# hG3n/mvStereoVision3

Measured on AMD Instinct MI355X. Metric: Mpix disparities/sec (SGBM 128-disp, 8-path) at 1/2/4/8 GPUs; % HBM roofline, higher is better.
Workload: dtype int16; 1 GPU; sgbm_1280x960_d128_8path_batch8; width=1280, height=960, num_disparities=128, min_disparity=1, block_size=13, mode=MODE_HH, frames_per_gpu=8, global_batch=8, params=configs/sgbm.yml + mode, gather=none, launch=single process, batches_in_flight=2, parallelism=frame-parallel x1

## Files before the change

mvstereovision3_amd/csrc/mvsv_bsgm.hip:

```cpp
#include <algorithm>
#include <cstdio>
#include <cstdlib>
#include <cstring>
#include <type_traits>
#include <vector>

#include "mvsv_bitslice.hpp"
#include "mvsv_device.hpp"
#include "mvsv_internal.hpp"

namespace mvsv {

using namespace dev;

namespace {

constexpr uint32_t kOnes = 0xffffffffu;

__device__ __forceinline__ uint32_t xswap(uint32_t v)
{
    return (uint32_t)__builtin_amdgcn_mov_dpp((int)v, 0xB1, 0xf, 0xf, true);
}

template <int P1, int P2>
// ... 571 lines not shown
        const int xl = x - dlo, xh = x - dhi;
        auto d2at = [&](int xx) -> int {
            const uint32_t kk = __hip_atomic_load(krow + xx, __ATOMIC_RELAXED, __HIP_MEMORY_SCOPE_AGENT);
            if (kk == 0xffffffffu) return INV;
            const int xc = 0xffff - (int)(kk & 0xffffu);
            return xc + minX1 - xx;
        };
        if (0 <= xl && xl < W && 0 <= xh && xh < W) {
            const int a = d2at(xl), b = d2at(xh);
            if (a >= minD && abs(a - dlo) > e.disp12 && b >= minD && abs(b - dhi) > e.disp12)
                orow[x] = (int16_t)INV;
        }
    }
}

constexpr int kBsWtaThreads = 512;

template <bool SIDE, int NDIR>
__global__ __launch_bounds__(kBsWtaThreads) void bsgm_wta_kernel(const uint32_t* __restrict__ Bc,
                                                                 const uint32_t* __restrict__ A, size_t aplane,
                                                                 const uint32_t* __restrict__ Dl, size_t dplane,
                                                                 const int16_t* __restrict__ C,
                                                                 const uint16_t* __restrict__ Mv, int H, int W,
                                                                 SgbmEff e, int16_t* __restrict__ raw,
                                                                 uint32_t* __restrict__ keys)
{
    static_assert(NDIR == 8 || NDIR == 5, "8 or 5 directions");
    const int y = blockIdx.x, f = blockIdx.y;
    const int W1 = e.W1;
    const int INV = e.invalid;
    const bool lane_rule = NDIR == 5 && !(e.variant & MVSV_VARIANT_WTA_MIN_D);
    int16_t* orow = raw + ((size_t)f * H + y) * W;
    uint32_t* krow = keys + ((size_t)f * H + y) * W;
    for (int x = threadIdx.x; x < W; x += kBsWtaThreads) {
        orow[x] = (int16_t)INV;
        krow[x] = 0xffffffffu;
    }
    __threadfence_block();
    __syncthreads();
    const int h = threadIdx.x & 1;
    const size_t pix0 = ((size_t)f * H + y) * W1;
    for (int xb = 0; xb < W1; xb += kBsWtaThreads / 2) {
        const int xr = xb + (threadIdx.x >> 1);
        const bool own = xr < W1;
        const int x = min(xr, W1 - 1);
        const size_t pix = pix0 + x;
        uint32_t c[2][4];
        uint32_t S[2][7];
        const size_t rowq = (size_t)(f * H + y) * bs::padq(W1);
        const uint32_t* qc = Bc + bs::cq_word(rowq, x, 2 * h);
        if constexpr (SIDE) {
#pragma unroll
            for (int e2 = 0; e2 < 2; e2++) {
                const uint4 t = *(const uint4*)(qc + 16 * e2);
                c[e2][0] = t.x, c[e2][1] = t.y, c[e2][2] = t.z, c[e2][3] = t.w;
                uint32_t dd[NDIR][3];
#pragma unroll
                for (int i = 0; i < NDIR; i++) {
                    const uint32_t* qd = Dl + (size_t)i * dplane + bs::dl_word(rowq, x, 2 * h + e2);
#pragma unroll
                    for (int b = 0; b < 3; b++) dd[i][b] = qd[b];
                }
                uint32_t a4[4][4], a5[2][5], s6[6];
                bs::add33(dd[0], dd[1], a4[0]);
                bs::add33(dd[2], dd[3], a4[1]);
                bs::add44(a4[0], a4[1], a5[0]);
                if constexpr (NDIR == 8) {
                    bs::add33(dd[4], dd[5], a4[2]);
                    bs::add33(dd[6], dd[7], a4[3]);
                    bs::add44(a4[2], a4[3], a5[1]);
                    bs::add55(a5[0], a5[1], s6);
                    bs::total8(c[e2], s6, S[e2]);
                } else {
                    const uint32_t d4[4] = {dd[4][0], dd[4][1], dd[4][2], 0u};
                    bs::add54(a5[0], d4, s6);
                    const uint32_t s5[5] = {s6[0], s6[1], s6[2], s6[3], s6[4]};
                    bs::total5(c[e2], s5, S[e2]);
                }
            }
        } else {
            const uint4* qd = (const uint4*)(A + pix * 16 + h * 8);
            const uint4* qu = (const uint4*)(A + aplane + pix * 16 + h * 8);
            const uint32_t* ql = Dl + bs::dl_word(rowq, x, 2 * h);
            const uint32_t* qr = Dl + dplane + bs::dl_word(rowq, x, 2 * h);
#pragma unroll
            for (int e2 = 0; e2 < 2; e2++) {
                uint4 t = *(const uint4*)(qc + 16 * e2);
                c[e2][0] = t.x, c[e2][1] = t.y, c[e2][2] = t.z, c[e2][3] = t.w;
                uint32_t ad[4], dl[3], dr[3];
                t = qd[e2];
                ad[0] = t.x, ad[1] = t.y, ad[2] = t.z, ad[3] = t.w;
#pragma unroll
                for (int b = 0; b < 3; b++) {
                    dl[b] = ql[12 * e2 + b];
                    dr[b] = qr[12 * e2 + b];
                }
                uint32_t d4[4];
                bs::add33(dl, dr, d4);
                if constexpr (NDIR == 8) {
                    uint32_t au[4], s5[5], s6[6];
                    t = qu[e2];
                    au[0] = t.x, au[1] = t.y, au[2] = t.z, au[3] = t.w;
                    bs::add44(ad, au, s5);
                    bs::add54(s5, d4, s6);
                    bs::total8(c[e2], s6, S[e2]);
                } else {
                    uint32_t s5[5];
                    bs::add44(ad, d4, s5);
                    bs::total5(c[e2], s5, S[e2]);
                }
            }
        }
        constexpr int TOP = NDIR == 8 ? 5 : 4;
        uint32_t kE = NDIR == 8 ? ~S[0][6] : ~(S[0][6] | S[0][5]);
        uint32_t kO = NDIR == 8 ? ~S[1][6] : ~(S[1][6] | S[1][5]);
        int mins = 0;
#pragma unroll
        for (int b = TOP; b >= 0; b--) {
            const uint32_t zE = bs::lop3<bs::kAndNotAB>(S[0][b], kE, kE);
            const uint32_t zO = bs::lop3<bs::kAndNotAB>(S[1][b], kO, kO);
            uint32_t any = zE | zO;
            any |= xswap(any);
            const bool fz = any != 0u;
            kE = fz ? zE : kE;
            kO = fz ? zO : kO;
            mins |= fz ? 0 : 1 << b;
        }
        int key = min(bs::wta_key(kE, h, 0, lane_rule), bs::wta_key(kO, h, 1, lane_rule));
        key = min(key, (int)xswap((uint32_t)key));
        const int best = key & 127;
        const int eb = best & 1;
        int Sm = 0, Sp = 0;
        {
            const int pm = ((best - 1 - 64 * h) >> 1) & 31, pp = ((best + 1 - 64 * h) >> 1) & 31;
#pragma unroll
            for (int b = 0; b < 7; b++) {
                const uint32_t wv = eb ? S[0][b] : S[1][b];
                Sm |= (int)(__builtin_amdgcn_ubfe(wv, (uint32_t)pm, 1u) << b);
                Sp |= (int)(__builtin_amdgcn_ubfe(wv, (uint32_t)pp, 1u) << b);
            }
            const int Smo = (int)xswap((uint32_t)Sm), Spo = (int)xswap((uint32_t)Sp);
            if (((best - 1) >> 6) != h) Sm = Smo;
            if (((best + 1) >> 6) != h) Sp = Spo;
        }
        if (h == 0 && own) bs_finish_pixel(C, Mv, pix, W1, W, x, best, mins, Sm, Sp, e, orow, krow);
    }
    __threadfence_block();
    __syncthreads();
    bs_lr_check_row(orow, krow, W, e, kBsWtaThreads);
}

constexpr int kBsRG = 3;

template <int P1, int P2, int NDIR>
__global__ __launch_bounds__(64) void bsgm_rlwta_kernel(const uint32_t* __restrict__ Bc,
                                                         const uint32_t* __restrict__ A, size_t aplane,
                                                         const uint32_t* __restrict__ Dlr, int H, int W1,
                                                         uint32_t* __restrict__ rec, int lane_rule)
{
    static_assert(NDIR == 8 || NDIR == 5, "8 or 5 directions");
    const int lane = threadIdx.x;
    const int q = lane & 3, rr = lane >> 2;
    const int y = min((int)blockIdx.x * 16 + rr, H - 1);
    const int f = blockIdx.y;
    const int h = q >> 1, eo = q & 1;
    const bool odd = eo != 0;
    const uint32_t fill_hi = q == 3 ? kOnes : 0u, fill_lo = q == 0 ? kOnes : 0u, sh = odd ? 1u : 31u;
    const size_t rowq = (size_t)(f * H + y) * bs::padq(W1);
    const size_t pixrow = (size_t)(f * H + y) * W1;
    const uint4* cgrp = (const uint4*)(Bc + bs::cq_word(rowq, 0, q));
    const uint4* dgrp = (const uint4*)(Dlr + bs::dl_word(rowq, 0, q));
    const uint4* adn = (const uint4*)(A + pixrow * 16 + 4 * q);
    const uint4* aup = (const uint4*)(A + aplane + pixrow * 16 + 4 * q);
    uint4* rgrp = (uint4*)(rec + rowq);
    const int G = (W1 + 3) >> 2;
    const int part = W1 & 3;
    auto grp = [&](int i) { return max(G - 1 - i, 0); };
    struct Ops {
        uint4 c[4], d[3], a[4], b[4];
    };
    auto load = [&](Ops& o, int i) {
        const int g = grp(i);
#pragma unroll
        for (int u = 0; u < 4; u++) o.c[u] = cgrp[(size_t)g * 16 + u];
#pragma unroll
        for (int u = 0; u < 3; u++) o.d[u] = dgrp[(size_t)g * 12 + u];
#pragma unroll
        for (int u = 0; u < 4; u++) {
            const int x = min(4 * g + u, W1 - 1);
            o.a[u] = adn[(size_t)x * 4];
            if constexpr (NDIR == 8) o.b[u] = aup[(size_t)x * 4];
        }
    };
    const int ph = part ? 1 : 0;
    Ops c0, ring[kBsRG];
    if (ph) load(c0, 0);
#pragma unroll
    for (int j = 0; j < kBsRG; j++) {
        load(ring[j], ph + j);
        __builtin_amdgcn_sched_barrier(0);
    }
    uint32_t st[3] = {0u, 0u, 0u};
    auto w4 = [](const uint4& v, int i) { return i == 0 ? v.x : i == 1 ? v.y : i == 2 ? v.z : v.w; };
    auto group = [&](int i, Ops& o, int n) {
        uint32_t rv[4];
#pragma unroll
        for (int k = 0; k < 4; k++) {
            const int u = 3 - k;
            if (u < n) {
                const uint32_t cw[4] = {o.c[u].x, o.c[u].y, o.c[u].z, o.c[u].w};
                uint32_t nw[3], dr[3];
                bs_quad_step<P1, P2>(st, cw, fill_hi, fill_lo, odd, sh, nw, dr);
#pragma unroll
                for (int b = 0; b < 3; b++) st[b] = nw[b];
                const uint32_t ad[4] = {o.a[u].x, o.a[u].y, o.a[u].z, o.a[u].w};
                uint32_t dl[3];
#pragma unroll
                for (int b = 0; b < 3; b++) dl[b] = w4(o.d[(3 * u + b) >> 2], (3 * u + b) & 3);
                uint32_t d4[4], S[7];
                bs::add33(dl, dr, d4);
                if constexpr (NDIR == 8) {
                    const uint32_t au[4] = {o.b[u].x, o.b[u].y, o.b[u].z, o.b[u].w};
                    uint32_t s5[5], s6[6];
                    bs::add44(ad, au, s5);
                    bs::add54(s5, d4, s6);
                    bs::total8(cw, s6, S);
                } else {
                    uint32_t s5[5];
                    bs::add44(ad, d4, s5);
                    bs::total5(cw, s5, S);
                }
                constexpr int TOP = NDIR == 8 ? 5 : 4;
                uint32_t kk = NDIR == 8 ? ~S[6] : ~(S[6] | S[5]);
                int mins = 0;
#pragma unroll
                for (int b = TOP; b >= 0; b--) {
                    const uint32_t z = bs::lop3<bs::kAndNotAB>(S[b], kk, kk);
                    uint32_t any = z | xswap(z);
                    any |= (uint32_t)__builtin_amdgcn_mov_dpp((int)any, 0x4E, 0xf, 0xf, true);
                    const bool fz = any != 0u;
                    kk = fz ? z : kk;
                    mins |= fz ? 0 : 1 << b;
                }
                int key = bs::wta_key(kk, h, eo, NDIR == 5 && lane_rule);
                key = min(key, (int)xswap((uint32_t)key));
                key = min(key, __builtin_amdgcn_mov_dpp(key, 0x4E, 0xf, 0xf, true));
                const int best = key & 127;
                auto sat = [&](int d) -> uint32_t {
                    const int dq = 2 * ((d >> 6) & 1) + (d & 1), p = ((d & 63) >> 1);
                    uint32_t v = 0;
#pragma unroll
                    for (int b = 0; b < 7; b++) v |= __builtin_amdgcn_ubfe(S[b], (uint32_t)p, 1u) << b;
                    return dq == q ? v : 0u;
                };
                uint32_t sm = sat(best - 1) | (sat(best + 1) << 8);
                sm |= xswap(sm);
                sm |= (uint32_t)__builtin_amdgcn_mov_dpp((int)sm, 0x4E, 0xf, 0xf, true);
                rv[u] = (uint32_t)best | ((uint32_t)mins << 8) | (sm << 16);
            } else {
                rv[u] = 0u;
            }
        }
        rgrp[grp(i)] = make_uint4(rv[0], rv[1], rv[2], rv[3]);
    };
    auto ringstep = [&](int i, int j, int n) {
        group(i, ring[j], n);
        load(ring[j], i + kBsRG);
        __builtin_amdgcn_sched_barrier(0);
    };
    if (ph) group(0, c0, part);
    int i = ph;
    for (; i + kBsRG <= G; i += kBsRG) {
#pragma unroll
        for (int j = 0; j < kBsRG; j++) ringstep(i + j, j, 4);
    }
#pragma unroll
    for (int j = 0; j < kBsRG; j++)
        if (i + j < G) ringstep(i + j, j, 4);
}

constexpr int kBsFinThreads = 256;
__global__ __launch_bounds__(kBsFinThreads) void bsgm_rl_final_kernel(const uint32_t* __restrict__ rec,
                                                                      const int16_t* __restrict__ C,
                                                                      const uint16_t* __restrict__ Mv, int H, int W,
                                                                      SgbmEff e, int16_t* __restrict__ raw,
                                                                      uint32_t* __restrict__ keys)
{
    const int y = blockIdx.x, f = blockIdx.y;
    const int W1 = e.W1;
    int16_t* orow = raw + ((size_t)f * H + y) * W;
    uint32_t* krow = keys + ((size_t)f * H + y) * W;
    for (int x = threadIdx.x; x < W; x += kBsFinThreads) {
        orow[x] = (int16_t)e.invalid;
        krow[x] = 0xffffffffu;
    }
    __threadfence_block();
    __syncthreads();
    const uint32_t* rrow = rec + (size_t)(f * H + y) * bs::padq(W1);
    const size_t pix0 = ((size_t)f * H + y) * W1;
    for (int x = threadIdx.x; x < W1; x += kBsFinThreads) {
        const uint32_t r = rrow[x];
        bs_finish_pixel(C, Mv, pix0 + x, W1, W, x, (int)(r & 0xffu), (int)((r >> 8) & 0xffu),
                        (int)((r >> 16) & 0xffu), (int)(r >> 24), e, orow, krow);
    }
    __threadfence_block();
    __syncthreads();
    bs_lr_check_row(orow, krow, W, e, kBsFinThreads);
}

__global__ __launch_bounds__(256) void bsgm_fixup_bottom_kernel(uint32_t* __restrict__ Bc, int16_t* __restrict__ C,
                                                                uint16_t* __restrict__ Mv, int H, int W1, int ylast,
                                                                int ybot)
{
    const int y = ybot + blockIdx.y, f = blockIdx.z;
    const size_t W1q = (size_t)bs::padq(W1);
    const size_t i = (size_t)blockIdx.x * 256 + threadIdx.x;
    const size_t nb = W1q * 4, nc = W1q * 16;
    const size_t src = (size_t)f * H + ylast, dst = (size_t)f * H + y;
    if (i < nb) {
        ((uint4*)Bc)[dst * nb + i] = ((const uint4*)Bc)[src * nb + i];
    } else if (i < nb + nc) {
        const size_t j = i - nb;
        ((uint4*)C)[dst * nc + j] = ((const uint4*)C)[src * nc + j];
    }
    if (i < (size_t)W1) Mv[dst * W1 + i] = Mv[src * W1 + i];
}

__global__ __launch_bounds__(128) void bsgm_fixup_col0_kernel(uint32_t* __restrict__ Bc, int16_t* __restrict__ C,
                                                              uint16_t* __restrict__ Mv, int H, int W1)
{
    const int y = 1 + blockIdx.x, f = blockIdx.y;
    const size_t W1q = (size_t)bs::padq(W1);
    const size_t r0 = (size_t)f * H, r = r0 + y;
    const int t = threadIdx.x;
    if (t < 16) {
        const int o = (t >> 2) * 16 + (t & 3);
        Bc[bs::cq_word(r * W1q, 0, 0) + o] = Bc[bs::cq_word(r0 * W1q, 0, 0) + o];
    }
    C[(r * W1q) * 128 + t * 4] = C[(r0 * W1q) * 128 + t * 4];
    if (t == 0) Mv[r * W1] = Mv[r0 * W1];
}

}

template <int NG>
static int launch_bs_strips(mvsv_ctx* ctx, const SgbmPlan& plan, int n, int H, const SgbmEff& e, const uint32_t* Bv,
                            uint32_t* Av, size_t aplane, uint32_t* dummy)
{
    using Cfg = BsStripCfg<NG>;
    int rc;
    unsigned epoch;
    long long ticket0;
    if ((rc = strip_begin(ctx, ctx->bs_bnd, 32, &epoch, &ticket0))) return rc;
    const dim3 grid((unsigned)plan.blocks);
    unsigned long long* stats = ctx->opt.bs_stats ? strip_stats_alloc(ctx, (size_t)grid.x * 64) : nullptr;
    const size_t lds = std::max(Cfg::kBytes, (size_t)(ctx->opt.bs_ldspad >= 0 ? ctx->opt.bs_ldspad : kBsStripLds));
    if (lds > 65536 &&
        (rc = check_hip(ctx, hipFuncSetAttribute((const void*)bsgm_strip_kernel<NG, 2, 5>,
                                                 hipFuncAttributeMaxDynamicSharedMemorySize, (int)lds),
                        "bit-sliced strip LDS attribute")))
        return rc;
    hipLaunchKernelGGL((bsgm_strip_kernel<NG, 2, 5>), grid, dim3(Cfg::kThreads), lds, ctx->stream, Bv, Av,
                       aplane, dummy, H, e.W1, plan.passes, (unsigned long long*)ctx->bs_bnd.ptr, epoch, n,
                       (int*)ctx->status.ptr, ctx->opt.spin_limit, ctx->report_target, ticket0, stats, 0);
    rc = check_hip(ctx, hipGetLastError(), "bit-sliced strip kernel");
    if (rc == MVSV_OK && ticket0 >= 0) ctx->tri_tickets += grid.x;
    std::vector<unsigned long long> hv;
    if (stats && strip_stats_read(ctx, stats, (size_t)grid.x * 8, &hv)) {
        unsigned long long t0 = ~0ull, t1 = 0, spin = 0, busy = 0, steps = 0;
        for (size_t b = 0; b < grid.x; b++) {
            const unsigned long long* q = &hv[b * 8];
            if (!q[1]) continue;
            t0 = std::min(t0, q[0]);
            t1 = std::max(t1, q[1]);
            spin += q[2];
            busy += q[1] - q[0];
            steps += q[4];
        }
        std::fprintf(stderr, "[bs] NG %d strips %d blocks %u span %llu ticks, block-ticks %llu, spin %.1f%%, ticks/step %.1f\n",
                     NG, plan.nstrips, grid.x, t1 - t0, busy, 100.0 * spin / std::max(busy, 1ull),
                     (double)busy / std::max(steps, 1ull));
    }
    return rc;
}

static int bsgm_paths_side(mvsv_ctx* ctx, const SgbmPlan& plan, int n, int H, int W, const SgbmEff& e,
                           const int16_t* Cv, const uint32_t* Bv, const uint16_t* Mv, int16_t* raw)
{
    int rc;
    const int npass = e.fullDP ? 2 : 1, ndir = plan.nplanes;
    const size_t dplane = plan.bs_dplane;
    uint32_t* Dv = (uint32_t*)ctx->agg.ptr;
    hipStream_t s = ctx->stream;
    {
        StageTimer tm(ctx, kStagePath);
        hipLaunchKernelGGL((bsgm_dir_kernel<2, 5>), dim3((e.W1 + H - 1 + 15) / 16, n, ndir), dim3(64), 0, s, Bv,
                           Dv, dplane, H, e.W1, Dv + ndir * dplane, npass);
        if ((rc = check_hip(ctx, hipGetLastError(), "bit-sliced direction kernel"))) return rc;
    }
    StageTimer tm(ctx, kStageFinal);
    if (e.fullDP)
        hipLaunchKernelGGL((bsgm_wta_kernel<true, 8>), dim3(H, n), dim3(kBsWtaThreads), 0, s, Bv, nullptr, (size_t)0,
                           Dv, dplane, Cv, Mv, H, W, e, raw, (uint32_t*)ctx->keys.ptr);
    else
        hipLaunchKernelGGL((bsgm_wta_kernel<true, 5>), dim3(H, n), dim3(kBsWtaThreads), 0, s, Bv, nullptr, (size_t)0,
                           Dv, dplane, Cv, Mv, H, W, e, raw, (uint32_t*)ctx->keys.ptr);
    return check_hip(ctx, hipGetLastError(), "bit-sliced WTA kernel");
}

int bsgm_cost_fixup(mvsv_ctx* ctx, int n, int H, const SgbmEff& e, int16_t* Cv, uint32_t* Bv, uint16_t* Mv)
{
    if (e.fullDP || H <= 1) return MVSV_OK;
    hipStream_t s = ctx->stream;
    const int ybot = std::max(H - e.SH2, 1), ylast = std::max(H - e.SH2 - 1, 0);
    StageTimer tm(ctx, kStageFixup);
    if (ybot < H) {
        const size_t items = (size_t)bs::padq(e.W1) * 20;
        hipLaunchKernelGGL(bsgm_fixup_bottom_kernel, dim3((unsigned)((items + 255) / 256), H - ybot, n), dim3(256),
                           0, s, Bv, Cv, Mv, H, e.W1, ylast, ybot);
    }
    if (!(e.variant & MVSV_VARIANT_FIRSTCOL_FIX))
        hipLaunchKernelGGL(bsgm_fixup_col0_kernel, dim3(H - 1, n), dim3(128), 0, s, Bv, Cv, Mv, H, e.W1);
    return check_hip(ctx, hipGetLastError(), "bit-sliced cost fixup");
}

int bsgm_paths(mvsv_ctx* ctx, const SgbmPlan& plan, int n, int H, int W, const SgbmEff& e, const int16_t* Cv,
               const uint32_t* Bv, const uint16_t* Mv, int16_t* raw)
{
    int rc;
    if (plan.sched == 2) return bsgm_paths_side(ctx, plan, n, H, W, e, Cv, Bv, Mv, raw);
    const int npass = plan.passes;
    const size_t aplane = plan.bs_aplane, dplane = plan.bs_dplane;
    uint32_t* Av = (uint32_t*)ctx->agg.ptr;
    uint32_t* Dv = Av + npass * aplane;
    hipStream_t s = ctx->stream;
    if ((rc = ensure_aux(ctx))) return rc;
    {
        StageTimer tm(ctx, kStagePath);
        const bool side = plan.lines_aux != 0;
        if (side && ((rc = check_hip(ctx, hipEventRecord(ctx->ev_fork, s), "fork")) ||
                     (rc = check_hip(ctx, hipStreamWaitEvent(ctx->aux, ctx->ev_fork, 0), "fork wait"))))
            return rc;
        hipStream_t ls = side ? ctx->aux : s;
        const bool fuse = ctx->opt.bs_fuse != 0;
        auto lines = [&]() -> int {
            StageTimer tl(ctx, kStageLines, ls);
            hipLaunchKernelGGL((bsgm_lines4_kernel<2, 5>), dim3((H + 15) / 16, n, fuse ? 1 : 2), dim3(64), 0, ls,
                               Bv, Dv, dplane, H, e.W1);
            return check_hip(ctx, hipGetLastError(), "bit-sliced line kernel");
        };
        if (side && (rc = lines())) return rc;
        {
            StageTimer ts(ctx, kStageStrips);
            uint32_t* dummy = Dv + 2 * dplane;
            switch (plan.bs_groups) {
            case 1: rc = launch_bs_strips<1>(ctx, plan, n, H, e, Bv, Av, aplane, dummy); break;
            case 2: rc = launch_bs_strips<2>(ctx, plan, n, H, e, Bv, Av, aplane, dummy); break;
            case 3: rc = launch_bs_strips<3>(ctx, plan, n, H, e, Bv, Av, aplane, dummy); break;
            case 4: rc = launch_bs_strips<4>(ctx, plan, n, H, e, Bv, Av, aplane, dummy); break;
            case 5: rc = launch_bs_strips<5>(ctx, plan, n, H, e, Bv, Av, aplane, dummy); break;
            default: rc = set_error(ctx, MVSV_E_HIP, "internal: no bit-sliced strip kernel of the SGBM plan's width");
            }
            if (rc) return rc;
        }
        if (!side && (rc = lines())) return rc;
        if (side && ((rc = check_hip(ctx, hipEventRecord(ctx->ev_join, ctx->aux), "join")) ||
                     (rc = check_hip(ctx, hipStreamWaitEvent(s, ctx->ev_join, 0), "join wait"))))
            return rc;
    }
    StageTimer tm(ctx, kStageFinal);
    if (ctx->opt.bs_fuse) {
        uint32_t* rec = Dv + dplane;
        const int lane_rule = !(e.variant & MVSV_VARIANT_WTA_MIN_D);
        if (e.fullDP)
            hipLaunchKernelGGL((bsgm_rlwta_kernel<2, 5, 8>), dim3((H + 15) / 16, n), dim3(64), 0, s, Bv, Av, aplane,
                               Dv, H, e.W1, rec, lane_rule);
        else
            hipLaunchKernelGGL((bsgm_rlwta_kernel<2, 5, 5>), dim3((H + 15) / 16, n), dim3(64), 0, s, Bv, Av, aplane,
                               Dv, H, e.W1, rec, lane_rule);
        if ((rc = check_hip(ctx, hipGetLastError(), "bit-sliced R->L + WTA kernel"))) return rc;
        hipLaunchKernelGGL(bsgm_rl_final_kernel, dim3(H, n), dim3(kBsFinThreads), 0, s, rec, Cv, Mv, H, W, e, raw,
                           (uint32_t*)ctx->keys.ptr);
        return check_hip(ctx, hipGetLastError(), "bit-sliced final kernel");
    }
    if (e.fullDP)
        hipLaunchKernelGGL((bsgm_wta_kernel<false, 8>), dim3(H, n), dim3(kBsWtaThreads), 0, s, Bv, Av, aplane, Dv,
                           dplane, Cv, Mv, H, W, e, raw, (uint32_t*)ctx->keys.ptr);
    else
        hipLaunchKernelGGL((bsgm_wta_kernel<false, 5>), dim3(H, n), dim3(kBsWtaThreads), 0, s, Bv, Av, aplane, Dv,
                           dplane, Cv, Mv, H, W, e, raw, (uint32_t*)ctx->keys.ptr);
    return check_hip(ctx, hipGetLastError(), "bit-sliced WTA kernel");
}

}
```

mvstereovision3_amd/csrc/mvsv_host.cpp:

```cpp
#include <algorithm>
#include <cerrno>
#include <cmath>
#include <cstdio>
#include <cstdlib>
#include <cstring>
#include <fstream>
#include <functional>
#include <map>
#include <sstream>
#include <string>

#include "mvsv_internal.hpp"

namespace mvsv {

int set_error(mvsv_ctx* ctx, int code, const std::string& msg)
{
    if (ctx) ctx->err = msg;
    return code;
}

int check_hip(mvsv_ctx* ctx, hipError_t e, const char* what)
{
    if (e == hipSuccess) return MVSV_OK;
// ... 187 lines not shown

}

using namespace mvsv;

static void drop_graphs(mvsv_ctx* ctx)
{
    for (auto& g : ctx->graph_cache)
        if (g.exec) (void)hipGraphExecDestroy(g.exec);
    ctx->graph_cache.clear();
    ctx->graph_seen.clear();
}

constexpr size_t kGraphCache = 4;
static int graph_run(mvsv_ctx* ctx, const std::vector<unsigned char>& key, const std::function<int()>& body)
{
    for (auto& g : ctx->graph_cache) {
        if (g.key != key) continue;
        if (g.epoch == ctx->alloc_epoch) {
            g.used = ++ctx->graph_clock;
            return check_hip(ctx, hipGraphLaunch(g.exec, ctx->stream), "graph launch");
        }
        (void)hipGraphExecDestroy(g.exec);
        g.exec = nullptr;
        g.key.clear();
    }
    if (ctx->graph_seen != key) {
        ctx->graph_seen = key;
        return body();
    }
    static const bool dbg = std::getenv("MVSV_GRAPH_DEBUG") != nullptr;
    auto fail = [&]() {
        const hipError_t le = hipGetLastError();
        if (dbg) std::fprintf(stderr, "[mvsv graph] capture failed (%s); graphs off for this context\n",
                              hipGetErrorString(le));
        ctx->graphs = 0;
        ctx->graph_seen.clear();
        return body();
    };
    if (!ctx->cap && hipStreamCreateWithFlags(&ctx->cap, hipStreamNonBlocking) != hipSuccess) return fail();
    const unsigned ep = ctx->alloc_epoch;
    if (hipStreamBeginCapture(ctx->cap, hipStreamCaptureModeRelaxed) != hipSuccess) return fail();
    hipStream_t keep = ctx->stream;
    ctx->stream = ctx->cap;
    const int rc = body();
    ctx->stream = keep;
    hipGraph_t graph = nullptr;
    const hipError_t ce = hipStreamEndCapture(ctx->cap, &graph);
    hipGraphExec_t exec = nullptr;
    const bool ok = rc == MVSV_OK && ce == hipSuccess && graph && ctx->alloc_epoch == ep &&
                    hipGraphInstantiate(&exec, graph, nullptr, nullptr, 0) == hipSuccess;
    if (graph) (void)hipGraphDestroy(graph);
    if (!ok) return fail();
    auto slot = ctx->graph_cache.end();
    for (auto it = ctx->graph_cache.begin(); it != ctx->graph_cache.end(); ++it)
        if (!it->exec) slot = it;
    if (slot == ctx->graph_cache.end() && ctx->graph_cache.size() >= kGraphCache) {
        slot = std::min_element(ctx->graph_cache.begin(), ctx->graph_cache.end(),
                                [](const mvsv_ctx::GraphEntry& a, const mvsv_ctx::GraphEntry& b) {
                                    return a.used < b.used;
                                });
        (void)hipGraphExecDestroy(slot->exec);
    }
    if (slot == ctx->graph_cache.end()) {
        ctx->graph_cache.emplace_back();
        slot = ctx->graph_cache.end() - 1;
    }
    slot->key = key;
    slot->exec = exec;
    slot->epoch = ep;
    slot->used = ++ctx->graph_clock;
    ctx->graph_seen.clear();
    if (dbg)
        std::fprintf(stderr, "[mvsv graph] captured a %zu-byte key, %zu cached\n", key.size(),
                     ctx->graph_cache.size());
    return check_hip(ctx, hipGraphLaunch(exec, ctx->stream), "graph launch");
}

template <typename T>
static void key_put(std::vector<unsigned char>& k, const T& v)
{
    const unsigned char* p = reinterpret_cast<const unsigned char*>(&v);
    k.insert(k.end(), p, p + sizeof(T));
}

extern "C" {

int mvsv_sgbm_validate(const mvsv_sgbm_params* p, int W, int H)
{
    SgbmEff e;
    std::string why;
    return resolve_sgbm(p, W, H, &e, &why);
}

int mvsv_bm_validate(const mvsv_bm_params* p, int W, int H)
{
    BmEff e;
    std::string why;
    return resolve_bm(p, W, H, &e, &why);
}

int mvsv_create(mvsv_ctx** out, int hip_device)
{
    if (!out) return MVSV_E_INVALID_ARG;
    *out = nullptr;
    int count = 0;
    if (hipGetDeviceCount(&count) != hipSuccess || count <= 0) {
        (void)hipGetLastError();
        return MVSV_E_NODEV;
    }
    if (hip_device < 0 || hip_device >= count) return MVSV_E_INVALID_ARG;
    mvsv_ctx* c = new (std::nothrow) mvsv_ctx();
    if (!c) return MVSV_E_OOM;
    c->device = hip_device;
    DeviceGuard dev_guard(hip_device);
    if (hipStreamCreateWithFlags(&c->own, hipStreamNonBlocking) != hipSuccess ||
        hipEventCreateWithFlags(&c->ev_last, hipEventDisableTiming) != hipSuccess ||
        alloc_report(c, 1, &c->report, &c->report_dev) != MVSV_OK) {
        (void)hipGetLastError();
        if (c->ev_last) (void)hipEventDestroy(c->ev_last);
        if (c->own) (void)hipStreamDestroy(c->own);
        delete c;
        return MVSV_E_HIP;
    }
    c->report_target = c->report_dev;
    c->stream = c->own;
    if (const char* v = std::getenv("MVSV_STRIP_SPIN_LIMIT"))
        c->opt.spin_limit = (unsigned)std::strtoul(v, nullptr, 0);
    if (const char* v = std::getenv("MVSV_KERNELS")) {
        if (std::strstr(v, "cost-lds")) c->opt.cost2 = 0;
        if (std::strstr(v, "path-wave")) c->opt.path16 = 0;
        if (std::strstr(v, "path-lines")) c->opt.tri = 0;
        if (std::strstr(v, "bm-tile")) c->opt.bm2 = 0;
        if (std::strstr(v, "cost-generic")) c->opt.cost_fixed_pp = 0;
    }
    if (const char* v = std::getenv("MVSV_COST_TY")) c->opt.cost_ty = std::max(0, std::atoi(v));
    if (const char* v = std::getenv("MVSV_PATH_SCHEDULE")) c->opt.path_sched = std::max(0, std::min(2, std::atoi(v)));
    if (const char* v = std::getenv("MVSV_STRIP_WAVES")) c->opt.strip_waves = std::max(0, std::atoi(v));
    if (const char* v = std::getenv("MVSV_TRI32")) c->opt.tri32 = std::atoi(v) != 0;
    if (const char* v = std::getenv("MVSV_FINAL_SPLIT")) c->opt.final_split = std::atoi(v) != 0;
    if (const char* v = std::getenv("MVSV_COST_RESIDUAL")) c->opt.cost_res = std::atoi(v) != 0;
    if (const char* v = std::getenv("MVSV_BM_TY")) c->opt.bm_ty = std::max(0, std::min(128, std::atoi(v)));
    if (hipDeviceGetAttribute(&c->cus, hipDeviceAttributeMultiprocessorCount, hip_device) != hipSuccess) {
        (void)hipGetLastError();
        c->cus = 256;
    }
    if (const char* v = std::getenv("MVSV_STRIP_ORDER")) c->opt.strip_tickets = std::strcmp(v, "blockidx") != 0;
    if (const char* v = std::getenv("MVSV_LINES_AUX")) c->opt.lines_aux = std::max(-1, std::min(2, std::atoi(v)));
    if (const char* v = std::getenv("MVSV_BITSLICE")) c->opt.bitslice = std::atoi(v) != 0;
    if (const char* v = std::getenv("MVSV_GRAPHS")) c->graphs = std::atoi(v) != 0;
    if (const char* v = std::getenv("MVSV_BS_SERIAL")) c->opt.bs_serial = std::atoi(v) != 0;
    if (const char* v = std::getenv("MVSV_COST_XCD")) c->opt.cost_xcd = std::atoi(v) != 0;
    if (const char* v = std::getenv("MVSV_BS_FUSE")) c->opt.bs_fuse = std::atoi(v) != 0;
    c->opt.tri_stats = std::getenv("MVSV_TRI_STATS") != nullptr;
    if (const char* v = std::getenv("MVSV_TRI_TRACE")) c->opt.tri_trace = v;
    c->opt.bs_stats = std::getenv("MVSV_BS_STATS") != nullptr;
    if (const char* v = std::getenv("MVSV_BS_LDSPAD")) c->opt.bs_ldspad = std::max(0L, std::atol(v));
    if (const char* v = std::getenv("MVSV_BS_GROUPS")) {
        const int g = std::atoi(v);
        c->opt.bs_groups = (g >= 1 && g <= 5) ? g : 0;
    }
    *out = c;
    return MVSV_OK;
}

static void free_buf(DevBuf& b)
{
    if (b.ptr) (void)hipFree(b.ptr);
    b.ptr = nullptr;
    b.bytes = 0;
}

int mvsv_trim(mvsv_ctx* ctx)
{
    if (!ctx) return MVSV_E_INVALID_ARG;
    ++ctx->alloc_epoch;
    DeviceGuard dev_guard(ctx->device);
    (void)hipStreamSynchronize(ctx->stream);
    DevBuf* all[] = {&ctx->pre, &ctx->cost, &ctx->cres, &ctx->agg, &ctx->raw, &ctx->uf_parent, &ctx->uf_size, &ctx->uf_lroot, &ctx->uf_list,
                     &ctx->uf_tile, &ctx->tri_bnd, &ctx->bs_bnd, &ctx->status,
                     &ctx->dummy, &ctx->keys,
                     &ctx->bm_lf, &ctx->bm_rf, &ctx->bm_cost, &ctx->bm_sad, &ctx->h_left, &ctx->h_right,
                     &ctx->h_out, &ctx->mm_part, &ctx->cl_rows, &ctx->sh_part, &ctx->ud_maps};
    for (DevBuf* b : all) free_buf(*b);
    ctx->ud_key.clear();
    return MVSV_OK;
}

static const char* kStageNames[MVSV_NUM_STAGES] = {
    "prefilter", "cost_volume", "cost_fixup", "path_aggregation", "final_wta_lr", "post_filters",
    "bm_match", "path_strips", "path_lines"};

const char* mvsv_profile_stage_name(int s)
{
    return (s >= 0 && s < MVSV_NUM_STAGES) ? kStageNames[s] : "";
}

int mvsv_profile_enable(mvsv_ctx* ctx, int on)
{
    if (!ctx) return MVSV_E_INVALID_ARG;
    ctx->prof = on ? 1 : 0;
    return MVSV_OK;
}

int mvsv_profile_reset(mvsv_ctx* ctx)
{
    if (!ctx) return MVSV_E_INVALID_ARG;
    (void)hipStreamSynchronize(ctx->stream);
    for (auto& m : ctx->marks) {
        ctx->event_pool.push_back(m.a);
        ctx->event_pool.push_back(m.b);
    }
    ctx->marks.clear();
    return MVSV_OK;
}

int mvsv_profile_read(mvsv_ctx* ctx, double* ms, int* launches, int n)
{
    if (!ctx || n < 0) return MVSV_E_INVALID_ARG;
    DeviceGuard dev_guard(ctx->device);
    int rc = check_hip(ctx, hipStreamSynchronize(ctx->stream), "hipStreamSynchronize");
    if (rc) return rc;
    for (int i = 0; i < n; i++) {
        if (ms) ms[i] = 0.0;
        if (launches) launches[i] = 0;
    }
    for (auto& m : ctx->marks) {
        if (m.stage >= n) continue;
        float t = 0.f;
        if (hipEventElapsedTime(&t, m.a, m.b) != hipSuccess) {
            (void)hipGetLastError();
            continue;
        }
        if (ms) ms[m.stage] += t;
        if (launches) launches[m.stage] += 1;
    }
    return MVSV_OK;
}

void mvsv_destroy(mvsv_ctx* ctx)
{
    if (!ctx) return;
    drop_graphs(ctx);
    mvsv_trim(ctx);
    if (ctx->cap) (void)hipStreamDestroy(ctx->cap);
    mvsv_profile_reset(ctx);
    for (hipEvent_t e : ctx->event_pool) (void)hipEventDestroy(e);
    if (ctx->ev_fork) (void)hipEventDestroy(ctx->ev_fork);
    if (ctx->ev_join) (void)hipEventDestroy(ctx->ev_join);
    if (ctx->ev_last) (void)hipEventDestroy(ctx->ev_last);
    if (ctx->report) (void)hipHostFree(ctx->report);
    if (ctx->aux) (void)hipStreamDestroy(ctx->aux);
    if (ctx->own) (void)hipStreamDestroy(ctx->own);
    delete ctx;
}

const char* mvsv_last_error(const mvsv_ctx* ctx) { return ctx ? ctx->err.c_str() : "null context"; }

static int switch_stream(mvsv_ctx* ctx, hipStream_t s)
{
    if (s == ctx->stream) return MVSV_OK;
    DeviceGuard dev_guard(ctx->device);
    if (ctx->last_valid) {
        int rc = check_hip(ctx, hipStreamWaitEvent(s, ctx->ev_last, 0), "stream switch wait");
        if (rc) return rc;
    }
    ctx->stream = s;
    return MVSV_OK;
}

int mvsv_set_stream(mvsv_ctx* ctx, void* s)
{
    if (!ctx) return MVSV_E_INVALID_ARG;
    return switch_stream(ctx, (hipStream_t)s);
}

int mvsv_use_own_stream(mvsv_ctx* ctx)
{
    if (!ctx) return MVSV_E_INVALID_ARG;
    return switch_stream(ctx, ctx->own);
}

int mvsv_set_option(mvsv_ctx* ctx, int option, long long value)
{
    if (!ctx) return MVSV_E_INVALID_ARG;
    switch (option) {
    case MVSV_OPT_STRIP_SPIN_LIMIT:
        if (value < 0 || value > 0xffffffffLL)
            return set_error(ctx, MVSV_E_INVALID_ARG, "spin limit must be 0..2^32-1");
        ctx->opt.spin_limit = (unsigned)value;
        return MVSV_OK;
    case MVSV_OPT_BM_TILE_ROWS:
        if (value < 0 || value > 128) return set_error(ctx, MVSV_E_INVALID_ARG, "BM tile rows must be 0..128");
        ctx->opt.bm_ty = (int)value;
        return MVSV_OK;
    case MVSV_OPT_PATH_SCHEDULE:
        if (value < 0 || value > 2) return set_error(ctx, MVSV_E_INVALID_ARG, "path schedule must be 0..2");
        ctx->opt.path_sched = (int)value;
        return MVSV_OK;
    case MVSV_OPT_STRIP_WAVES:
        if (value < 0 || value > 64) return set_error(ctx, MVSV_E_INVALID_ARG, "strip waves must be 0..64");
        ctx->opt.strip_waves = (int)value;
        return MVSV_OK;
    case MVSV_OPT_STRIP_TICKETS:
        if (value < 0 || value > 1) return set_error(ctx, MVSV_E_INVALID_ARG, "strip tickets must be 0 or 1");
        ctx->opt.strip_tickets = (int)value;
// ... 765 lines not shown
```

mvstereovision3_amd/csrc/mvsv_sgbm_plan.hpp:

```cpp
#pragma once

#include <cstddef>
#include <cstdint>
#include <string>

#include "mvsv_bitslice.hpp"
#include "mvsv_cost_layout.hpp"

namespace mvsv {

constexpr int kPlanBitslice = 1, kPlanSide = 2, kPlanStrips = 4, kPlanResidual = 8;

struct SgbmEff {
    int minD, maxD, D;
    int SW2, SH2;
    int ftzero;
    int uniq, disp12;
    int P1, P2;
    int minX1, maxX1, W1;
    int invalid;
    int fullDP;
    int variant;
    int speckle_window, speckle_diff;
    int cn;
};

constexpr unsigned kStripSpinLimitDefault = 1u << 20;

struct KernelOptions {
    int strip_tickets = 1;
    unsigned spin_limit = kStripSpinLimitDefault;
    int path16 = 1;
    int cost2 = 1;
    int cost_fixed_pp = 1;
    int cost_ty = 0;
    int tri = 1;
    int path_sched = 0;
    int tri32 = 1;
    int final_split = 1;
    int strip_waves = 0;
    int cost_res = 1;
    int lines_aux = -1;
    int bitslice = 1;
    int bs_groups = 0;
    int cost_xcd = 1;
    int bs_fuse = 1;
    int bs_serial = 0;
    int bm2 = 1;
    int bm_ty = 0;
    int tri_stats = 0;
    std::string tri_trace;
    int bs_stats = 0;
    long bs_ldspad = -1;
};

constexpr int tri_wide_waves(int np, int lpc) { return lpc == 8 ? 7 : (np >= 8 ? 7 : 15); }
constexpr int tri_narrow_waves(int np, int lpc) { return lpc == 8 ? 4 : lpc == 32 ? 8 : (np >= 8 ? 4 : 8); }
constexpr int tri_strip_cols(int waves, int lpc) { return (64 / lpc) * waves; }
constexpr int tri_granules(int np) { return (2 * np + 3) / 3; }
constexpr int bs_strip_cols(int groups) { return 32 * groups; }
constexpr int kBsGran = 36;

constexpr int ceil_div(int a, int b) { return (a + b - 1) / b; }
constexpr size_t align256(size_t b) { return (b + 255) & ~(size_t)255; }

inline bool sgbm_no_wrap(const SgbmEff& e)
{
    const long bs = 2L * e.SW2 + 1;
    return (long)e.P2 + bs * bs * e.cn * (2L * e.ftzero + 63) + e.P2 <= 32767;
}

MVSV_HD inline bool acc_is_u8(const SgbmEff& e) { return (e.fullDP ? 8 : 5) * e.P2 <= 255; }
MVSV_HD inline bool acc_is_nib(const SgbmEff& e) { return 3 * e.P2 <= 15; }

struct Cost2Launch {
    bool fits;
    int stg, ppc;
    size_t lds;
    Cost2Layout l;
};
inline Cost2Launch cost2_launch(const SgbmEff& e, int fixed_pp, int TY)
{
    Cost2Launch c{};
    if (e.SH2 > 7 || e.SW2 != e.SH2 || e.D < 2 || e.D / 2 > kCost2Threads) return c;
    c.l = cost2_layout(e.D, e.SW2, TY);
    const int items = 2 * c.l.NX + e.D - 1;
    c.stg = items > kCost2Threads ? 2 : 1;
    c.ppc = !fixed_pp ? 0 : c.l.PP == 64 ? 64 : (c.l.PP == 128 ? 128 : 0);
    c.lds = cost2_total_bytes(c.l, 2 * e.SH2 + 1, c.stg, c.ppc);
    c.fits = c.l.CL >= 1 && items <= kCost2Threads * 2 && c.lds <= 160 * 1024;
    return c;
}
inline bool cost2_runs(const KernelOptions& o, const SgbmEff& e)
{
    return e.cn == 1 && o.cost2 && cost2_launch(e, o.cost_fixed_pp, kCostTileHeights[0]).fits;
}

inline bool bsgm_eligible(const KernelOptions& o, const SgbmEff& e, int n, int H)
{
    return e.cn == 1 && o.bitslice && e.D == 128 && e.P1 == 2 && e.P2 == 5 && e.uniq == 0 && sgbm_no_wrap(e) &&
           e.W1 > 0 && (size_t)n * H * bs::padq(e.W1) * 16 < ((size_t)1 << 31);
}

inline bool wta_split(const KernelOptions& o, const SgbmEff& e) { return o.final_split && e.P2 > 15 && e.D <= 32; }

inline bool use_residual(const KernelOptions& o, const SgbmEff& e, int sched)
{
    return e.cn == 1 && o.cost_res && (sched == 1 || sched == 2) && sgbm_no_wrap(e) && 3 * e.P2 <= 15 &&
           (e.D == 32 || e.D == 64 || e.D == 128);
}

inline bool use_strips(const KernelOptions& o, const SgbmEff& e, int H)
{
    return o.tri && (size_t)H * e.W1 * e.D < ((size_t)1 << 31);
}

inline int path_schedule(const KernelOptions& o, int cus, const SgbmEff& e, int H, int n)
{
    if (e.D == 16 && o.path16 && o.path_sched != 1) return 2;
    if (!o.path16 || !(e.D == 32 || e.D == 64 || e.D == 128 || e.D == 256)) return 0;
    const bool dirs_ok = e.P2 <= 15 || o.path_sched == 2;
    if (o.path_sched == 2) return 2;
    if (o.path_sched == 0 && bsgm_eligible(o, e, n, H) && e.SH2 <= 7 && e.SW2 == e.SH2) {
        const long long dirpix = (long long)n * e.W1 * H * (e.fullDP ? 8 : 5);
        if (dirpix <= 12000000LL) return 2;
        return use_strips(o, e, H) ? 1 : 0;
    }
    if (o.path_sched == 0 && dirs_ok) {
        const int wide = e.D > 128 ? 7 : 15;
        const long long blocks = (long long)(e.fullDP ? 2 : 1) * n * ((e.W1 + H - 1 + 4 * wide - 1) / (4 * wide));
        if (2 * blocks <= cus) return 2;
    }
    if (o.path_sched == 0 && e.P2 > 15) {
        const double bytes = (double)n * e.W1 * H * e.D * (e.fullDP ? 7 : 4) * (acc_is_u8(e) ? 1 : 2);
        if (bytes <= 1.4e9) return 2;
    }
    return use_strips(o, e, H) ? 1 : 0;
}

inline int cost_tile_height(const KernelOptions& o, int cus, const SgbmEff& e, int n, int H)
{
    if (o.cost_ty > 0) return o.cost_ty;
    if (H < 256) return 16;
    const int TX = cost2_layout(e.D, e.SW2, 120).TX;
    const long tiles_x = (e.W1 + TX - 1) / TX;
    auto tiles = [&](int ty) { return tiles_x * ((H + ty - 1) / ty) * n; };
    int TY = 120;
    if (tiles(120) < 1024) {
        long best = -1;
        for (int ty : kCostTileHeights) {
            const long per_cu = (tiles(ty) + cus - 1) / cus;
            const long c = per_cu * (ty + 2 * e.SH2) * (per_cu == 1 ? 3 : 2);
            if (best < 0 || c < best) {
                best = c;
                TY = ty;
            }
        }
    }
    return TY;
}

enum SgbmFamily {
    kFamGeneric = 0,
    kFamPacked16,
    kFamPacked8,
    kFamBitslice
};
enum SgbmAcc { kAccNib = 4, kAccU8 = 8, kAccU16 = 16, kAccWords = 32 };

struct SgbmPlan {
    bool empty = true;
    int family = kFamGeneric;
    int sched = 0;
    bool cost2 = false;
    int cost_ty = 16;
    bool residual = false;
    bool no_wrap = false;
    bool nw = false;
    int acc = kAccU16;
    int nplanes = 1;
    bool split = false;
    int passes = 0;
    int lpc = 0;
    int waves = 0;
    int bs_groups = 0;
    size_t bs_aplane = 0, bs_dplane = 0;
    int strip_cols = 0;
    int nstrips = 0;
    long long blocks = 0;
    int lines_aux = 0;
    size_t pre = 0, cost = 0, cres = 0, cres_min = 0 , agg = 0,
           raw = 0, keys = 0, dummy = 0, tri_bnd = 0, bs_bnd = 0, status = 0;

    size_t total_bytes() const
    {
        return pre + cost + cres + agg + raw + keys + dummy + tri_bnd + bs_bnd + status;
    }
    int bits() const
    {
// ... 103 lines not shown
```

Before: 3344 Mpix/s.

## Split R->L WTA kernel into producer wave and three consumer waves via LDS

Replaces the single-wave fused right-to-left path + WTA kernel with a 256-thread block. One wave runs the serial bit-sliced R->L recurrence and hands cost words and path results through a double-buffered LDS slot. Three consumer waves take every third group round-robin to do the totals, argmin and record output. The goal is to take the WTA work off the serial dependency chain so it runs in parallel with it. The cost is many block barriers per group, LDS traffic, and a producer wave that still bounds throughput. The old kernel is kept behind an env flag, and the new path is on by default.

```diff
diff --git a/mvstereovision3_amd/csrc/mvsv_bsgm.hip b/mvstereovision3_amd/csrc/mvsv_bsgm.hip
--- a/mvstereovision3_amd/csrc/mvsv_bsgm.hip
+++ b/mvstereovision3_amd/csrc/mvsv_bsgm.hip
@@ -747,11 +747,67 @@
 
 constexpr int kBsRG = 3;
 
+template <int NDIR>
+__device__ __forceinline__ void bs_rl_totals(const uint32_t (&cw)[4], const uint32_t (&ad)[4],
+                                             const uint32_t (&au)[4], const uint32_t (&dl)[3],
+                                             const uint32_t (&dr)[3], uint32_t (&S)[7])
+{
+    uint32_t d4[4];
+    bs::add33(dl, dr, d4);
+    if constexpr (NDIR == 8) {
+        uint32_t s5[5], s6[6];
+        bs::add44(ad, au, s5);
+        bs::add54(s5, d4, s6);
+        bs::total8(cw, s6, S);
+    } else {
+        uint32_t s5[5];
+        bs::add44(ad, d4, s5);
+        bs::total5(cw, s5, S);
+    }
+}
+
+template <int NDIR>
+__device__ __forceinline__ void bs_rl_argmin(const uint32_t (&S)[7], int h, int eo, bool lane_rule, int& best,
+                                             int& mins)
+{
+    constexpr int TOP = NDIR == 8 ? 5 : 4;
+    uint32_t kk = NDIR == 8 ? ~S[6] : ~(S[6] | S[5]);
+    mins = 0;
+#pragma unroll
+    for (int b = TOP; b >= 0; b--) {
+        const uint32_t z = bs::lop3<bs::kAndNotAB>(S[b], kk, kk);
+        uint32_t any = z | xswap(z);
+        any |= (uint32_t)__builtin_amdgcn_mov_dpp((int)any, 0x4E, 0xf, 0xf, true);
+        const bool fz = any != 0u;
+        kk = fz ? z : kk;
+        mins |= fz ? 0 : 1 << b;
+    }
+    int key = bs::wta_key(kk, h, eo, NDIR == 5 && lane_rule);
+    key = min(key, (int)xswap((uint32_t)key));
+    key = min(key, __builtin_amdgcn_mov_dpp(key, 0x4E, 0xf, 0xf, true));
+    best = key & 127;
+}
+
+__device__ __forceinline__ uint32_t bs_rl_record(const uint32_t (&S)[7], int best, int mins, int q)
+{
+    auto sat = [&](int d) -> uint32_t {
+        const int dq = 2 * ((d >> 6) & 1) + (d & 1), p = ((d & 63) >> 1);
+        uint32_t v = 0;
+#pragma unroll
+        for (int b = 0; b < 7; b++) v |= __builtin_amdgcn_ubfe(S[b], (uint32_t)p, 1u) << b;
+        return dq == q ? v : 0u;
+    };
+    uint32_t sm = sat(best - 1) | (sat(best + 1) << 8);
+    sm |= xswap(sm);
+    sm |= (uint32_t)__builtin_amdgcn_mov_dpp((int)sm, 0x4E, 0xf, 0xf, true);
+    return (uint32_t)best | ((uint32_t)mins << 8) | (sm << 16);
+}
+
 template <int P1, int P2, int NDIR>
-__global__ __launch_bounds__(64) void bsgm_rlwta_kernel(const uint32_t* __restrict__ Bc,
-                                                         const uint32_t* __restrict__ A, size_t aplane,
-                                                         const uint32_t* __restrict__ Dlr, int H, int W1,
-                                                         uint32_t* __restrict__ rec, int lane_rule)
+__global__ __launch_bounds__(64) void bsgm_rlwta1_kernel(const uint32_t* __restrict__ Bc,
+                                                          const uint32_t* __restrict__ A, size_t aplane,
+                                                          const uint32_t* __restrict__ Dlr, int H, int W1,
+                                                          uint32_t* __restrict__ rec, int lane_rule)
 {
     static_assert(NDIR == 8 || NDIR == 5, "8 or 5 directions");
     const int lane = threadIdx.x;
@@ -812,46 +868,12 @@
                 uint32_t dl[3];
 #pragma unroll
                 for (int b = 0; b < 3; b++) dl[b] = w4(o.d[(3 * u + b) >> 2], (3 * u + b) & 3);
-                uint32_t d4[4], S[7];
-                bs::add33(dl, dr, d4);
-                if constexpr (NDIR == 8) {
-                    const uint32_t au[4] = {o.b[u].x, o.b[u].y, o.b[u].z, o.b[u].w};
-                    uint32_t s5[5], s6[6];
-                    bs::add44(ad, au, s5);
-                    bs::add54(s5, d4, s6);
-                    bs::total8(cw, s6, S);
-                } else {
-                    uint32_t s5[5];
-                    bs::add44(ad, d4, s5);
-                    bs::total5(cw, s5, S);
-                }
-                constexpr int TOP = NDIR == 8 ? 5 : 4;
-                uint32_t kk = NDIR == 8 ? ~S[6] : ~(S[6] | S[5]);
-                int mins = 0;
-#pragma unroll
-                for (int b = TOP; b >= 0; b--) {
-                    const uint32_t z = bs::lop3<bs::kAndNotAB>(S[b], kk, kk);
-                    uint32_t any = z | xswap(z);
-                    any |= (uint32_t)__builtin_amdgcn_mov_dpp((int)any, 0x4E, 0xf, 0xf, true);
-                    const bool fz = any != 0u;
-                    kk = fz ? z : kk;
-                    mins |= fz ? 0 : 1 << b;
-                }
-                int key = bs::wta_key(kk, h, eo, NDIR == 5 && lane_rule);
-                key = min(key, (int)xswap((uint32_t)key));
-                key = min(key, __builtin_amdgcn_mov_dpp(key, 0x4E, 0xf, 0xf, true));
-                const int best = key & 127;
-                auto sat = [&](int d) -> uint32_t {
-                    const int dq = 2 * ((d >> 6) & 1) + (d & 1), p = ((d & 63) >> 1);
-                    uint32_t v = 0;
-#pragma unroll
-                    for (int b = 0; b < 7; b++) v |= __builtin_amdgcn_ubfe(S[b], (uint32_t)p, 1u) << b;
-                    return dq == q ? v : 0u;
-                };
-                uint32_t sm = sat(best - 1) | (sat(best + 1) << 8);
-                sm |= xswap(sm);
-                sm |= (uint32_t)__builtin_amdgcn_mov_dpp((int)sm, 0x4E, 0xf, 0xf, true);
-                rv[u] = (uint32_t)best | ((uint32_t)mins << 8) | (sm << 16);
+                uint32_t au[4] = {0u, 0u, 0u, 0u}, S[7];
+                if constexpr (NDIR == 8) au[0] = o.b[u].x, au[1] = o.b[u].y, au[2] = o.b[u].z, au[3] = o.b[u].w;
+                bs_rl_totals<NDIR>(cw, ad, au, dl, dr, S);
+                int best, mins;
+                bs_rl_argmin<NDIR>(S, h, eo, lane_rule != 0, best, mins);
+                rv[u] = bs_rl_record(S, best, mins, q);
             } else {
                 rv[u] = 0u;
             }
@@ -872,6 +894,216 @@
 #pragma unroll
     for (int j = 0; j < kBsRG; j++)
         if (i + j < G) ringstep(i + j, j, 4);
+}
+
+constexpr int kBsPR = 6;
+constexpr int kBsCR = 2;
+using BsHand = uint4[7][64];
+
+__device__ __forceinline__ void bs_lds_barrier()
+{
+    asm volatile("s_waitcnt lgkmcnt(0)" ::: "memory");
+    __builtin_amdgcn_s_barrier();
+}
+
+template <int P1, int P2>
+__device__ __forceinline__ void bs_rlw_producer(const uint4* __restrict__ cgrp, int G, int part, int q, int lane,
+                                                BsHand* hand, int T)
+{
+    const bool odd = (q & 1) != 0;
+    const uint32_t fill_hi = q == 3 ? kOnes : 0u, fill_lo = q == 0 ? kOnes : 0u, sh = odd ? 1u : 31u;
+    auto grp = [&](int i) { return max(G - 1 - i, 0); };
+    struct Cg {
+        uint4 c[4];
+    };
+    auto load = [&](Cg& o, int i) {
+        const int g = grp(i);
+#pragma unroll
+        for (int u = 0; u < 4; u++) o.c[u] = cgrp[(size_t)g * 16 + u];
+    };
+    const int ph = part ? 1 : 0;
+    Cg c0, ring[kBsPR];
+    if (ph) load(c0, 0);
+#pragma unroll
+    for (int j = 0; j < kBsPR; j++) {
+        load(ring[j], ph + j);
+        __builtin_amdgcn_sched_barrier(0);
+    }
+    uint32_t st[3] = {0u, 0u, 0u};
+    auto group = [&](Cg& o, int n, uint4* dst) {
+        uint32_t dd[12];
+#pragma unroll
+        for (int k = 0; k < 4; k++) {
+            const int u = 3 - k;
+            if (u < n) {
+                const uint32_t cw[4] = {o.c[u].x, o.c[u].y, o.c[u].z, o.c[u].w};
+                uint32_t nw[3], dr[3];
+                bs_quad_step<P1, P2>(st, cw, fill_hi, fill_lo, odd, sh, nw, dr);
+#pragma unroll
+                for (int b = 0; b < 3; b++) st[b] = nw[b], dd[3 * u + b] = dr[b];
+            } else {
+#pragma unroll
+                for (int b = 0; b < 3; b++) dd[3 * u + b] = 0u;
+            }
+        }
+#pragma unroll
+        for (int u = 0; u < 4; u++) dst[u * 64] = o.c[u];
+#pragma unroll
+        for (int v = 0; v < 3; v++) dst[(4 + v) * 64] = make_uint4(dd[4 * v], dd[4 * v + 1], dd[4 * v + 2], dd[4 * v + 3]);
+    };
+    uint4* const slot[2] = {&hand[ph][0][lane], &hand[ph ^ 1][0][lane]};
+    if (ph) {
+        group(c0, part, &hand[0][0][lane]);
+        bs_lds_barrier();
+    }
+    int i = ph;
+    for (; i + kBsPR <= G; i += kBsPR) {
+#pragma unroll
+        for (int j = 0; j < kBsPR; j++) {
+            group(ring[j], 4, slot[j & 1]);
+            load(ring[j], i + j + kBsPR);
+            __builtin_amdgcn_sched_barrier(0);
+            bs_lds_barrier();
+        }
+    }
+#pragma unroll
+    for (int j = 0; j < kBsPR; j++)
+        if (i + j < G) {
+            group(ring[j], 4, slot[j & 1]);
+            bs_lds_barrier();
+        }
+    for (int nb = max(G, 0); nb < T; nb++) bs_lds_barrier();
+}
+
+template <int NDIR, int CW>
+__device__ __forceinline__ void bs_rlw_consumer(const uint4* __restrict__ dgrp, const uint4* __restrict__ adn,
+                                                const uint4* __restrict__ aup, uint4* __restrict__ rgrp, int G,
+                                                int part, int W1, int q, int lane, bool lane_rule,
+                                                const BsHand* hand, int T)
+{
+    static_assert(kBsCR == 2, "two own groups per trip: the slot parity of each is fixed");
+    constexpr int I0 = CW % 3;
+    const int h = q >> 1, eo = q & 1;
+    auto grp = [&](int i) { return max(G - 1 - i, 0); };
+    struct Ops {
+        uint4 d[3], a[4], b[4];
+    };
+    auto load = [&](Ops& o, int i) {
+        const int g = grp(i);
+#pragma unroll
+        for (int u = 0; u < 3; u++) o.d[u] = dgrp[(size_t)g * 12 + u];
+#pragma unroll
+        for (int u = 0; u < 4; u++) {
+            const int x = min(4 * g + u, W1 - 1);
+            o.a[u] = adn[(size_t)x * 4];
+            if constexpr (NDIR == 8) o.b[u] = aup[(size_t)x * 4];
+        }
+    };
+    Ops ring[kBsCR];
+#pragma unroll
+    for (int j = 0; j < kBsCR; j++) {
+        load(ring[j], I0 + 3 * j);
+        __builtin_amdgcn_sched_barrier(0);
+    }
+    auto w4 = [](const uint4& v, int i) { return i == 0 ? v.x : i == 1 ? v.y : i == 2 ? v.z : v.w; };
+    auto own = [&](int i, Ops& o, const uint4* src) {
+        uint4 hc[4], hd[3];
+#pragma unroll
+        for (int u = 0; u < 4; u++) hc[u] = src[u * 64];
+#pragma unroll
+        for (int v = 0; v < 3; v++) hd[v] = src[(4 + v) * 64];
+        uint32_t S[4][7];
+#pragma unroll
+        for (int u = 0; u < 4; u++) {
+            const uint32_t cw[4] = {hc[u].x, hc[u].y, hc[u].z, hc[u].w};
+            const uint32_t ad[4] = {o.a[u].x, o.a[u].y, o.a[u].z, o.a[u].w};
+            uint32_t au[4] = {0u, 0u, 0u, 0u}, dl[3], dr[3];
+            if constexpr (NDIR == 8) au[0] = o.b[u].x, au[1] = o.b[u].y, au[2] = o.b[u].z, au[3] = o.b[u].w;
+#pragma unroll
+            for (int b = 0; b < 3; b++) {
+                dl[b] = w4(o.d[(3 * u + b) >> 2], (3 * u + b) & 3);
+                dr[b] = w4(hd[(3 * u + b) >> 2], (3 * u + b) & 3);
+            }
+            bs_rl_totals<NDIR>(cw, ad, au, dl, dr, S[u]);
+        }
+        load(o, i + 3 * kBsCR);
+        __builtin_amdgcn_sched_barrier(0);
+        auto pinS = [&]() {
+#pragma unroll
+            for (int u = 0; u < 4; u++)
+                asm volatile("" : "+v"(S[u][0]), "+v"(S[u][1]), "+v"(S[u][2]), "+v"(S[u][3]), "+v"(S[u][4]),
+                                  "+v"(S[u][5]), "+v"(S[u][6]));
+        };
+        pinS();
+        bs_lds_barrier();
+        pinS();
+        int best[4], mins[4];
+#pragma unroll
+        for (int u = 0; u < 4; u++) bs_rl_argmin<NDIR>(S[u], h, eo, lane_rule, best[u], mins[u]);
+        auto pinB = [&]() {
+#pragma unroll
+            for (int u = 0; u < 4; u++) asm volatile("" : "+v"(best[u]), "+v"(mins[u]));
+        };
+        pinB();
+        bs_lds_barrier();
+        pinB();
+        const int n = (i == 0 && part) ? part : 4;
+        uint32_t rv[4];
+#pragma unroll
+        for (int u = 0; u < 4; u++) {
+            const uint32_t r = bs_rl_record(S[u], best[u], mins[u], q);
+            rv[u] = u < n ? r : 0u;
+        }
+        rgrp[grp(i)] = make_uint4(rv[0], rv[1], rv[2], rv[3]);
+        bs_lds_barrier();
+    };
+    for (int k = 0; k <= I0; k++) bs_lds_barrier();
+    const uint4* const s0 = &hand[I0 & 1][0][lane];
+    const uint4* const s1 = &hand[(I0 + 1) & 1][0][lane];
+    int i = I0;
+    for (; i + 3 < G; i += 6) {
+        own(i, ring[0], s0);
+        own(i + 3, ring[1], s1);
+    }
+    if (i < G) {
+        own(i, ring[0], s0);
+        i += 3;
+    }
+    for (int nb = i + 1; nb < T; nb++) bs_lds_barrier();
+}
+
+template <int P1, int P2, int NDIR>
+__global__ __launch_bounds__(256) void bsgm_rlwta_kernel(const uint32_t* __restrict__ Bc,
+                                                          const uint32_t* __restrict__ A, size_t aplane,
+                                                          const uint32_t* __restrict__ Dlr, int H, int W1,
+                                                          uint32_t* __restrict__ rec, int lane_rule)
+{
+    static_assert(NDIR == 8 || NDIR == 5, "8 or 5 directions");
+    __shared__ BsHand hand[2];
+    const int lane = threadIdx.x & 63;
+    const int wave = __builtin_amdgcn_readfirstlane((int)(threadIdx.x >> 6));
+    const int q = lane & 3, rr = lane >> 2;
+    const int y = min((int)blockIdx.x * 16 + rr, H - 1);
+    const int f = blockIdx.y;
+    const size_t rowq = (size_t)(f * H + y) * bs::padq(W1);
+    const size_t pixrow = (size_t)(f * H + y) * W1;
+    const uint4* cgrp = (const uint4*)(Bc + bs::cq_word(rowq, 0, q));
+    const uint4* dgrp = (const uint4*)(Dlr + bs::dl_word(rowq, 0, q));
+    const uint4* adn = (const uint4*)(A + pixrow * 16 + 4 * q);
+    const uint4* aup = (const uint4*)(A + aplane + pixrow * 16 + 4 * q);
+    uint4* rgrp = (uint4*)(rec + rowq);
+    const int G = (W1 + 3) >> 2;
+    const int part = W1 & 3;
+    const int T = G + 3;
+    const bool lr = lane_rule != 0;
+    if (wave == 0)
+        bs_rlw_producer<P1, P2>(cgrp, G, part, q, lane, hand, T);
+    else if (wave == 1)
+        bs_rlw_consumer<NDIR, 1>(dgrp, adn, aup, rgrp, G, part, W1, q, lane, lr, hand, T);
+    else if (wave == 2)
+        bs_rlw_consumer<NDIR, 2>(dgrp, adn, aup, rgrp, G, part, W1, q, lane, lr, hand, T);
+    else
+        bs_rlw_consumer<NDIR, 3>(dgrp, adn, aup, rgrp, G, part, W1, q, lane, lr, hand, T);
 }
 
 constexpr int kBsFinThreads = 256;
@@ -1067,12 +1299,22 @@
     if (ctx->opt.bs_fuse) {
         uint32_t* rec = Dv + dplane;
         const int lane_rule = !(e.variant & MVSV_VARIANT_WTA_MIN_D);
-        if (e.fullDP)
-            hipLaunchKernelGGL((bsgm_rlwta_kernel<2, 5, 8>), dim3((H + 15) / 16, n), dim3(64), 0, s, Bv, Av, aplane,
-                               Dv, H, e.W1, rec, lane_rule);
-        else
-            hipLaunchKernelGGL((bsgm_rlwta_kernel<2, 5, 5>), dim3((H + 15) / 16, n), dim3(64), 0, s, Bv, Av, aplane,
-                               Dv, H, e.W1, rec, lane_rule);
+        const dim3 rgrid((H + 15) / 16, n);
+        if (ctx->opt.bs_rlsplit) {
+            if (e.fullDP)
+                hipLaunchKernelGGL((bsgm_rlwta_kernel<2, 5, 8>), rgrid, dim3(256), 0, s, Bv, Av, aplane, Dv, H, e.W1,
+                                   rec, lane_rule);
+            else
+                hipLaunchKernelGGL((bsgm_rlwta_kernel<2, 5, 5>), rgrid, dim3(256), 0, s, Bv, Av, aplane, Dv, H, e.W1,
+                                   rec, lane_rule);
+        } else {
+            if (e.fullDP)
+                hipLaunchKernelGGL((bsgm_rlwta1_kernel<2, 5, 8>), rgrid, dim3(64), 0, s, Bv, Av, aplane, Dv, H, e.W1,
+                                   rec, lane_rule);
+            else
+                hipLaunchKernelGGL((bsgm_rlwta1_kernel<2, 5, 5>), rgrid, dim3(64), 0, s, Bv, Av, aplane, Dv, H, e.W1,
+                                   rec, lane_rule);
+        }
         if ((rc = check_hip(ctx, hipGetLastError(), "bit-sliced R->L + WTA kernel"))) return rc;
         hipLaunchKernelGGL(bsgm_rl_final_kernel, dim3(H, n), dim3(kBsFinThreads), 0, s, rec, Cv, Mv, H, W, e, raw,
                            (uint32_t*)ctx->keys.ptr);
diff --git a/mvstereovision3_amd/csrc/mvsv_host.cpp b/mvstereovision3_amd/csrc/mvsv_host.cpp
--- a/mvstereovision3_amd/csrc/mvsv_host.cpp
+++ b/mvstereovision3_amd/csrc/mvsv_host.cpp
@@ -363,6 +363,7 @@
     if (const char* v = std::getenv("MVSV_BS_SERIAL")) c->opt.bs_serial = std::atoi(v) != 0;
     if (const char* v = std::getenv("MVSV_COST_XCD")) c->opt.cost_xcd = std::atoi(v) != 0;
     if (const char* v = std::getenv("MVSV_BS_FUSE")) c->opt.bs_fuse = std::atoi(v) != 0;
+    if (const char* v = std::getenv("MVSV_BS_RLSPLIT")) c->opt.bs_rlsplit = std::atoi(v) != 0;
     c->opt.tri_stats = std::getenv("MVSV_TRI_STATS") != nullptr;
     if (const char* v = std::getenv("MVSV_TRI_TRACE")) c->opt.tri_trace = v;
     c->opt.bs_stats = std::getenv("MVSV_BS_STATS") != nullptr;
diff --git a/mvstereovision3_amd/csrc/mvsv_sgbm_plan.hpp b/mvstereovision3_amd/csrc/mvsv_sgbm_plan.hpp
--- a/mvstereovision3_amd/csrc/mvsv_sgbm_plan.hpp
+++ b/mvstereovision3_amd/csrc/mvsv_sgbm_plan.hpp
@@ -45,6 +45,7 @@
     int bs_groups = 0;
     int cost_xcd = 1;
     int bs_fuse = 1;
+    int bs_rlsplit = 1;
     int bs_serial = 0;
     int bm2 = 1;
     int bm_ty = 0;
```

Measured after the change: 3307 Mpix/s. 1.1% lower.
